# dluvizon/deephar

Hardware: NVIDIA H100
Metric: frames/sec (256x256, 16-frame clips, b32) (higher is better)
Workload: dtype bf16x3 split (fp32 accumulate, wgmma)

## Files before the change

### deephar_b200/csrc/conv_patch.cu

```cuda
#include "tc_common.cuh"

namespace tcd {
using namespace tc;
using R = tc::Roles<2>;
constexpr int WARP_EPI0 = R::WARP_EPI0, WARP_TMA = R::WARP_TMA, WARP_PATCH = R::WARP_PATCH, NTHREADS = R::NTHREADS,
              REGS_PROD = R::REGS_PROD, REGS_EPI = R::REGS_EPI, REGS_CTRL = R::REGS_CTRL;

constexpr int A_BYTES = BM * 64;
constexpr int NWG = 128;
constexpr int NA = 4;
constexpr int NB = 3;
constexpr int MAX_NP = 8;

struct PatchParams {
    TcParams t;
    int np, patch_stride, patch_bytes;
    int ntaps, ncb;
    int tw;
    int ry, fn;
    int pc, pr;
    int rows_per_frame;
    int kw;
    int pt, pl, sh, sw;
    int vh, vw;
    int mask;
};

template <bool LO>
__global__ void __launch_bounds__(NTHREADS, 1)
patch_dense_kernel(const __grid_constant__ PatchParams PP, const __grid_constant__ CUtensorMap map_hi,
                   const __grid_constant__ CUtensorMap map_lo, const __grid_constant__ CUtensorMap map_x) {
    const TcParams& P = PP.t;
    extern __shared__ __align__(1024) uint8_t smem_raw[];
    if (smem_u32(smem_raw) & 1023u) __trap();
    uint8_t* smem = smem_raw;
    const int tid = threadIdx.x;
    const int warp = tid >> 5, lane = tid & 31;
    constexpr bool want_lo = LO;
    const int b_bytes = P.bn_cta * 64;
    uint8_t* b_ring = smem + NA * 2 * A_BYTES;
    uint8_t* patch0 = b_ring + NB * 2 * b_bytes;
    uint64_t* bars = reinterpret_cast<uint64_t*>(patch0 + (size_t)PP.np * PP.patch_stride);
    constexpr int NB_A = NA + 2 * NA;
    constexpr int NB_P = NB_A + 2 * NB;
    const uint32_t bar_full0 = smem_u32(bars), bar_empty0 = smem_u32(bars + NA), bar_fullb0 = smem_u32(bars + NB_A),
                   bar_emptyb0 = smem_u32(bars + NB_A + NB), bar_pfull0 = smem_u32(bars + NB_P),
                   bar_pempty0 = smem_u32(bars + NB_P + MAX_NP);
    const int n0 = blockIdx.y * P.bn_cta;
    const int nkb = P.n_kblocks;
    const int ntaps = PP.ntaps, ncb = PP.ncb, np = PP.np;

    if (warp == WARP_TMA && lane == 0) {
        tma_prefetch_desc(&map_hi);
        if (want_lo) tma_prefetch_desc(&map_lo);
        tma_prefetch_desc(&map_x);
        for (int s = 0; s < NA; ++s) {
            mbar_init(bar_full0 + 8 * s, (uint32_t)NWG);
            mbar_init(bar_empty0 + 16 * s, (uint32_t)R::EPQ);
            mbar_init(bar_empty0 + 16 * s + 8, (uint32_t)R::EPQ);
        }
        for (int s = 0; s < NB; ++s) {
            mbar_init(bar_fullb0 + 8 * s, 1);
            mbar_init(bar_emptyb0 + 8 * s, R::EPQ);
        }
        for (int s = 0; s < MAX_NP; ++s) {
            mbar_init(bar_pfull0 + 8 * s, 1);
            mbar_init(bar_pempty0 + 8 * s, ntaps == 1 ? (uint32_t)NWG : (uint32_t)(2 * NWG));
        }
        fence_barrier_init();
    }
    __syncthreads();

    const int tiles_mine = ((int)P.n_mtiles - (int)blockIdx.x + (int)gridDim.x - 1) / (int)gridDim.x;
    const int total_g = tiles_mine * nkb;
    const int n_patches = tiles_mine * ncb;
    const int rows_per_tile = BM / PP.tw;

    if (warp < WARP_EPI0) {
        reg_prod<REGS_PROD, R::LAUNCH_REGS>();
        const ConvParams& c = P.c;
        const int w = warp >> 2;
        const int tw = tid & (NWG - 1);
        const int ch4 = tw & 7;
        const int prow = tw >> 3;
        uint32_t poff[8];
        int yy[8], xx[8];
// ... 74 lines not shown
                asm volatile("st.shared.v2.b32 [%0], {%1, %2};" ::"r"(a_hi + aoff[i]), "r"(h0), "r"(h1) : "memory");
                if (want_lo) asm volatile("st.shared.v2.b32 [%0], {%1, %2};" ::"r"(a_lo + aoff[i]), "r"(l0), "r"(l1) : "memory");
            }
            const bool last_of_patch = tap + 2 >= ntaps;
            if (last_of_patch) mbar_arrive(bar_pempty0 + 8 * slot);
            fence_proxy_async();
            mbar_arrive(bar_full0 + 8 * s);
            s += 2;
            if (s >= NA) { s -= NA; ++it; }
            tap += 2;
            kx += 2;
            while (tap >= ntaps) {
                tap -= ntaps;
                ++p;
                if (++cb == ncb) { cb = 0; ++ti; }
                if (++slot == np) { slot = 0; pphase ^= 1u; }
                ky = 0; kx = tap;
                if (kx >= PP.kw) { kx -= PP.kw; ky = 1; }
            }
            while (kx >= PP.kw) { kx -= PP.kw; ++ky; }
        }
    } else if (warp < WARP_TMA) {
        reg_inc<REGS_EPI>();
        const int wg = (warp - WARP_EPI0) >> 2, wt = tid - 32 * WARP_EPI0 - 128 * wg;
        float acc[R::MH][ACC_N];
        const uint64_t dbase = make_desc64(smem_u32(smem) + (uint32_t)(wg * 64 * 64));
        const uint64_t dbase_b = make_desc64(smem_u32(b_ring));
        const uint32_t sta16 = (2 * A_BYTES) >> 4, stb16 = (uint32_t)(2 * b_bytes) >> 4, alo16 = A_BYTES >> 4,
                       blo16 = (uint32_t)b_bytes >> 4;
        for (int ti = 0; ti < tiles_mine; ++ti) {
            const int g0 = ti * nkb;
            wg_tile<R::MH, SBK / 16, LO>(
                P.bn_cta, acc, nkb, 0u, alo16, blo16, true,
                [&](int kb, uint64_t& da, uint64_t& db) {
                    const int g = g0 + kb, s = g % NA, sb = g % NB;
                    mbar_wait(bar_full0 + 8 * s, (uint32_t)(g / NA) & 1);
                    mbar_wait(bar_fullb0 + 8 * sb, (uint32_t)(g / NB) & 1);
                    da = dbase + (uint64_t)((uint32_t)s * sta16);
                    db = dbase_b + (uint64_t)((uint32_t)sb * stb16);
                },
                [&](int kb) {
                    const int g = g0 + kb, s = g % NA;
                    wg_release<false>(bar_empty0 + 16 * s + 8 * ((g / NA) & 1), wg, wt, 0u);
                    if (wt == 0) mbar_arrive(bar_emptyb0 + 8 * (g % NB));
                });
            wg_epilogue<R::MH>(P, acc, ((int)blockIdx.x + ti * (int)gridDim.x) * BM + 64 * wg, n0, wt);
        }
    } else {
        reg_dec<REGS_CTRL>();
        if (warp == WARP_TMA) {
            if (lane == 0) {
                const uint32_t tx = (uint32_t)(want_lo ? 2 : 1) * (uint32_t)b_bytes;
                for (int g = 0; g < total_g; ++g) {
                    const int p = g / ntaps, tap = g - p * ntaps;
                    const int cb = p % ncb;
                    const int kc = tap * P.c.Cin + cb * SBK;
                    const int sb = g % NB;
                    const uint32_t itb = (uint32_t)(g / NB);
                    if (itb >= 1) mbar_wait_relaxed(bar_emptyb0 + 8 * sb, (itb - 1) & 1, 0u);
                    const uint32_t full = bar_fullb0 + 8 * sb;
                    mbar_arrive_expect_tx(full, tx);
                    const uint32_t b_hi = smem_u32(b_ring + (size_t)sb * (2 * b_bytes));
                    const uint32_t b_lo = b_hi + (uint32_t)b_bytes;
                    tma_load_2d(b_hi, &map_hi, kc, n0, full);
                    if (want_lo) tma_load_2d(b_lo, &map_lo, kc, n0, full);
                }
            }
        } else if (warp == WARP_PATCH) {
            if (lane == 0) {
// ... 39 lines not shown
    if (!(p.W == 128 || p.W == 64 || p.W == 32 || p.W == 16 || p.W == 8)) return false;
    const int tr = tc::BM / p.W;
    if (tr <= p.H ? (p.H % tr) != 0 : (tr % p.H) != 0) return false;
    g->tw = p.W;
    g->ry = tr <= p.H ? tr : p.H;
    g->fn = tr <= p.H ? 1 : tr / p.H;
    g->pc = p.W + p.kw - 1;
    g->pr = g->ry + p.kh - 1;
    g->rows_per_frame = p.H; g->vh = p.H; g->vw = p.W; g->vn = p.N;
    g->pt = p.pt; g->pl = p.pl; g->kw = p.kw; g->ntaps = p.kh * p.kw;
    g->w_stride = (int64_t)p.ldx * 4; g->h_stride = (int64_t)p.W * p.ldx * 4; g->n_stride = (int64_t)p.H * g->h_stride;
    return true;
}

template <bool LO>
static cudaError_t launch_patch(const PatchParams& PP, const CUtensorMap& map_hi, const CUtensorMap& map_lo,
                                const CUtensorMap& map_x, dim3 grid, size_t smem, cudaStream_t s) {
    cudaError_t e = tc::ensure_smem<patch_dense_kernel<LO>>(smem);
    if (e == cudaSuccess) patch_dense_kernel<LO><<<grid, NTHREADS, smem, s>>>(PP, map_hi, map_lo, map_x);
    return e;
}

static size_t fixed_smem(int bn_cta) {
    return (size_t)NA * 2 * A_BYTES + (size_t)NB * 2 * bn_cta * 64 + 512;
}

}

bool dh_patch_supported(const dh_ctx* ctx, const ConvParams& p, const dh_packed_w* packed) {
    using namespace tcd;
    if (!ctx->dense_patch) return false;
    if (!packed || !packed->hi || !packed->lo) return false;
    if (p.M < 1) return false;
    if ((p.Cin & 7) || (p.ldx & 3) || (reinterpret_cast<uintptr_t>(p.x) & 15)) return false;
    if (p.pre_scale && ((reinterpret_cast<uintptr_t>(p.pre_scale) & 15) || (reinterpret_cast<uintptr_t>(p.pre_shift) & 15)))
        return false;
    const int K = p.kh * p.kw * p.Cin;
    if (packed->k != dh_tc_k_pad(K) || packed->cout_pad != dh_tc_cout_pad(p.Cout)) return false;
    Geom g;
    if (!plan_geom(p, &g)) return false;
    if (g.pc > 256 || g.pr > 256 || g.fn > 256) return false;
    int bn_cta, gy;
    tc::tile_n(p.Cout, &bn_cta, &gy);
    const size_t patch = (size_t)tc::SBK * 4 * g.pc * g.pr * g.fn;
    const size_t stride = (patch + 1023) / 1024 * 1024;
    if (fixed_smem(bn_cta) + 2 * stride > 227 * 1024) return false;
    if ((g.w_stride & 15) || g.n_stride >= (1ll << 40)) return false;
// ... 70 lines not shown
```

### deephar_b200/csrc/conv_sep.cu

```cuda
#include "tc_common.cuh"

namespace tcs {
using namespace tc;
using R = tc::Roles<2, 1>;
constexpr int WARP_EPI0 = R::WARP_EPI0, WARP_TMA = R::WARP_TMA, WARP_PATCH = R::WARP_PATCH, NTHREADS = R::NTHREADS,
              REGS_PROD = R::REGS_PROD, REGS_EPI = R::REGS_EPI, REGS_CTRL = R::REGS_CTRL;

constexpr int A_BYTES = BM * 64;
constexpr int NWG = 128;
constexpr int NPW = 1;
constexpr int NA = 4;
constexpr int NB = 3;
constexpr int NP = 3;

struct SepParams {
    TcParams t;
    int patch_stride;
    int patch_bytes;
    int ry, fn;
    int dbg;
};

template <int KS, int TW, bool SHARE, bool BNPRO, bool LO>
__global__ void __launch_bounds__(NTHREADS, 1)
sep_tma_kernel(const __grid_constant__ SepParams SP, const __grid_constant__ CUtensorMap map_hi,
               const __grid_constant__ CUtensorMap map_lo, const __grid_constant__ CUtensorMap map_x) {
    constexpr int PAD = KS / 2;
    constexpr int PC = TW + 2 * PAD;
    constexpr int NR = 4 + KS - 1;
#ifdef DH_ABLATE
    const int DBG = SP.dbg;
#else
    constexpr int DBG = 0;
#endif
    const TcParams& P = SP.t;
    extern __shared__ __align__(1024) uint8_t smem_raw[];
    if (smem_u32(smem_raw) & 1023u) __trap();
    uint8_t* smem = smem_raw;
    const int tid = threadIdx.x;
    const int warp = tid >> 5, lane = tid & 31;
    constexpr bool want_lo = LO;
    const int b_bytes = P.bn_cta * 64;
    uint8_t* b_ring = smem + NA * 2 * A_BYTES;
    uint8_t* patch0 = b_ring + NB * 2 * b_bytes;
    uint64_t* bars = reinterpret_cast<uint64_t*>(patch0 + NP * SP.patch_stride);
    constexpr int NB_A = NA + 2 * NA;
    const uint32_t bar_full0 = smem_u32(bars), bar_empty0 = smem_u32(bars + NA), bar_fullb0 = smem_u32(bars + NB_A),
                   bar_emptyb0 = smem_u32(bars + NB_A + NB), bar_pfull0 = smem_u32(bars + NB_A + 2 * NB),
                   bar_pempty0 = smem_u32(bars + NB_A + 2 * NB + NP);
    const int n0 = blockIdx.y * P.bn_cta;
    const int nkb = P.n_kblocks;
    const uint32_t my_rank = SHARE ? cluster_ctarank() : 0u;

    if (warp == WARP_TMA && lane == 0) {
        tma_prefetch_desc(&map_hi);
        if (want_lo) tma_prefetch_desc(&map_lo);
        tma_prefetch_desc(&map_x);
        for (int s = 0; s < NA; ++s) {
            mbar_init(bar_full0 + 8 * s, SHARE ? 1u : (uint32_t)NWG);
            mbar_init(bar_empty0 + 16 * s, (SHARE ? 2u : 1u) * R::EPQ);
            mbar_init(bar_empty0 + 16 * s + 8, (SHARE ? 2u : 1u) * R::EPQ);
        }
        for (int s = 0; s < NB; ++s) {
            mbar_init(bar_fullb0 + 8 * s, 1);
            mbar_init(bar_emptyb0 + 8 * s, R::EPQ);
        }
        for (int s = 0; s < NP; ++s) {
            mbar_init(bar_pfull0 + 8 * s, 1);
            mbar_init(bar_pempty0 + 8 * s, NWG);
        }
        fence_barrier_init();
    }
    if (SHARE) cluster_sync_all(); else __syncthreads();

    const int tiles_mine = ((int)P.n_mtiles - (int)blockIdx.x + (int)gridDim.x - 1) / (int)gridDim.x;
    const int total_g = tiles_mine * nkb;
    const int n_own = SHARE ? (total_g - (int)my_rank + 1) / 2 : total_g;

    if (warp < WARP_EPI0) {
        reg_prod<REGS_PROD, R::LAUNCH_REGS>();
        const ConvParams& c = P.c;
        const int w = warp >> 2;
        const int tw = tid & (NWG - 1);
        const int cp = tw & 15;
        const int blk = tw >> 4;
        constexpr int XB = TW / 4;
        const int strip = blk / XB, xb = blk - strip * XB;
        const int fn = (strip * 4) / SP.ry, ry = (strip * 4) - fn * SP.ry;
// ... 94 lines not shown
                    split2(acc[o][q].x, acc[o][q].y, hi, lo);
                    const uint32_t off = swz64(row0 + o * TW + q, cp * 2);
                    *reinterpret_cast<uint32_t*>(a_hi + off) = hi;
                    if (want_lo) *reinterpret_cast<uint32_t*>(a_lo + off) = lo;
                }
            fence_proxy_async();
            if (SHARE) {
                asm volatile("bar.sync %0, %1;" ::"r"(1 + w), "r"(NWG) : "memory");
                if (tw == 0) {
                    mbar_arrive(bar_full0 + 8 * s);
                    const uint32_t peer = my_rank ^ 1u;
                    const uint32_t peer_full = mapa_peer(bar_full0 + 8 * s, peer);
                    if (!(DBG & 8)) {
                        bulk_s2peer(mapa_peer(smem_u32(a_hi), peer), smem_u32(a_hi), A_BYTES, peer_full);
                        if (want_lo) bulk_s2peer(mapa_peer(smem_u32(a_lo), peer), smem_u32(a_lo), A_BYTES, peer_full);
                    }
                }
            } else {
                mbar_arrive(bar_full0 + 8 * s);
            }
        }
    } else if (warp < WARP_TMA) {
        reg_inc<REGS_EPI>();
        const int wg = (warp - WARP_EPI0) >> 2, wt = tid - 32 * WARP_EPI0 - 128 * wg;
        float acc[R::MH][ACC_N];
        const uint64_t dbase = make_desc64(smem_u32(smem) + (uint32_t)(wg * 64 * 64));
        const uint64_t dbase_b = make_desc64(smem_u32(b_ring));
        const uint32_t sta16 = (2 * A_BYTES) >> 4, stb16 = (uint32_t)(2 * b_bytes) >> 4, alo16 = A_BYTES >> 4,
                       blo16 = (uint32_t)b_bytes >> 4;
        for (int ti = 0; ti < tiles_mine; ++ti) {
            const int g0 = ti * nkb;
            wg_tile<R::MH, SBK / 16, LO>(
                P.bn_cta, acc, nkb, 0u, alo16, blo16, !(DBG & 64),
                [&](int kb, uint64_t& da, uint64_t& db) {
                    const int g = g0 + kb, s = g % NA, sb = g % NB;
                    if (!(DBG & 128)) mbar_wait(bar_full0 + 8 * s, (uint32_t)(g / NA) & 1);
                    mbar_wait(bar_fullb0 + 8 * sb, (uint32_t)(g / NB) & 1);
                    da = dbase + (uint64_t)((uint32_t)s * sta16);
                    db = dbase_b + (uint64_t)((uint32_t)sb * stb16);
                },
                [&](int kb) {
                    const int g = g0 + kb, s = g % NA;
                    wg_release<SHARE>(bar_empty0 + 16 * s + 8 * ((g / NA) & 1), wg, wt, my_rank ^ 1u);
                    if (wt == 0) mbar_arrive(bar_emptyb0 + 8 * (g % NB));
                });
            wg_epilogue<R::MH>(P, acc, ((int)blockIdx.x + ti * (int)gridDim.x) * BM + 64 * wg, n0, wt);
        }
    } else {
        reg_dec<REGS_CTRL>();
        if (warp == WARP_TMA) {
            if (lane == 0) {
                const uint32_t tx = (DBG & 16) ? 0u : (uint32_t)(want_lo ? 2 : 1) * (uint32_t)b_bytes;
                const uint32_t tx_a = (DBG & 8) ? 0u : (uint32_t)(want_lo ? 2 : 1) * (uint32_t)A_BYTES;
                for (int g = 0; g < total_g; ++g) {
                    const int ti = g / nkb, kb = g - ti * nkb;
                    const int sb = g % NB;
                    const uint32_t itb = (uint32_t)(g / NB);
                    if (itb >= 1) mbar_wait_relaxed(bar_emptyb0 + 8 * sb, (itb - 1) & 1, (DBG & 2048) ? 64u : 0u);
                    const uint32_t full = bar_fullb0 + 8 * sb;
                    mbar_arrive_expect_tx(full, tx);
                    const uint32_t b_hi = smem_u32(b_ring + (size_t)sb * (2 * b_bytes));
                    const uint32_t b_lo = b_hi + (uint32_t)b_bytes;
                    if (!(DBG & 16)) {
                        tma_load_2d(b_hi, &map_hi, kb * SBK, n0, full);
                        if (want_lo) tma_load_2d(b_lo, &map_lo, kb * SBK, n0, full);
                    }
                    if (SHARE && (uint32_t)(g & 1) != my_rank) {
                        const int sa = g % NA;
                        wait_stage_free(bar_empty0, sa, (uint32_t)(g / NA));
// ... 72 lines not shown
    P.c.K = p.Cin;
    P.k_pad = packed->k;
    P.n_kblocks = p.Cin / SBK;
    int gy;
    tile_n(p.Cout, &P.bn_cta, &gy);
    P.precision = (precision == 1) ? 1 : 3;
    P.ks = p.kh;
    P.n_mtiles = (p.M + BM - 1) / BM;
    P.stages = 2;
    const int pad = p.kh / 2;
    const int tr = BM / p.W;
    SP.ry = tr <= p.H ? tr : p.H;
    SP.fn = tr <= p.H ? 1 : tr / p.H;
    const int pc = p.W + 2 * pad, prr = SP.ry + 2 * pad;
    SP.patch_bytes = SBK * 4 * pc * prr * SP.fn;
    SP.patch_stride = (SP.patch_bytes + 1023) / 1024 * 1024;
#ifdef DH_ABLATE
    SP.dbg = ctx->dbg;
    P.dbg = ctx->dbg;
#else
    SP.dbg = 0;
    P.dbg = 0;
#endif
    const size_t smem = (size_t)NA * 2 * A_BYTES + (size_t)NB * 2 * P.bn_cta * 64 + NP * (size_t)SP.patch_stride + 512;
    if (smem > 227 * 1024) {
        dh_set_error("dh_launch_sep_tma: tile does not fit shared memory");
        return -1;
    }
    CUtensorMap map_hi, map_lo, map_x;
    if (!make_map_b64(&map_hi, packed->hi, packed->k, packed->cout_pad, P.bn_cta) ||
        !make_map_b64(&map_lo, packed->lo, packed->k, packed->cout_pad, P.bn_cta) ||
        !make_map_x(&map_x, p, pc, prr, SP.fn)) {
        dh_set_error("dh_launch_sep_tma: cuTensorMapEncodeTiled failed");
        return -1;
    }
    int gx = ctx->num_sms / gy;
    if (gx < 1) gx = 1;
    if (gx > P.n_mtiles) gx = P.n_mtiles;
    dim3 grid(gx, gy);
    const bool share = gy % 2 == 0 && ctx->share_a;
    cudaError_t e = cudaSuccess;
#define DH_SEP_LAUNCH_(KS_, TW_, BN_, LO_)                                                                              \
    do {                                                                                                         \
        if (share) {                                                                                             \
            e = ensure_smem<sep_tma_kernel<KS_, TW_, true, BN_, LO_>>(smem); \
            if (e == cudaSuccess) {                                                                              \
                cudaLaunchConfig_t cfg = {};                                                                     \
// ... 29 lines not shown
```

### deephar_b200/csrc/conv_tc.cu

```cuda
#include "tc_common.cuh"

namespace tc {
using R = tc::Roles<1>;
constexpr int WARP_EPI0 = R::WARP_EPI0, WARP_TMA = R::WARP_TMA, NTHREADS = R::NTHREADS,
              REGS_PROD = R::REGS_PROD, REGS_EPI = R::REGS_EPI, REGS_CTRL = R::REGS_CTRL;

struct DenseRows {
    int base[8];
    int yx[8];
};

__device__ __forceinline__ void dense_rows_init(const ConvParams& c, int m0, int tid, DenseRows& R) {
    const int HoWo = c.Ho * c.Wo;
#pragma unroll
    for (int i = 0; i < 8; ++i) {
        const int m = m0 + (tid >> 4) + i * 16;
        if (m < c.M) {
            int n = m / HoWo;
            int rem = m - n * HoWo;
            int oy = rem / c.Wo;
            int ox = rem - oy * c.Wo;
            R.base[i] = n * c.H * c.W;
            R.yx[i] = ((oy * c.sh - c.pt) << 16) | ((ox * c.sw - c.pl) & 0xffff);
        } else {
// ... 209 lines not shown
            *reinterpret_cast<uint32_t*>(a_hi + off) = hi;
            if (want_lo) *reinterpret_cast<uint32_t*>(a_lo + off) = lo;
        }
}

__device__ __forceinline__ void dense_load_any(const TcParams& P, const DenseRows& R, int kb, int tid, DenseRegs& D) {
    if (P.ks < 0) dense_load_scalar(P, R, kb, tid, D);
    else dense_load(P, R, kb, tid, D);
}

template <int MODE, bool SHARE, bool LO>
__global__ void __launch_bounds__(NTHREADS, 1)
conv_tc_kernel(const __grid_constant__ TcParams P, const __grid_constant__ CUtensorMap map_hi,
               const __grid_constant__ CUtensorMap map_lo) {
    extern __shared__ __align__(1024) uint8_t smem_raw[];
    if (smem_u32(smem_raw) & 1023u) __trap();
    uint8_t* smem = smem_raw;
    const int tid = threadIdx.x;
    const int warp = tid >> 5, lane = tid & 31;
    constexpr bool want_lo = LO;
    const int b_tile_bytes = P.bn_cta * 128;
    const int stage_bytes = 2 * A_TILE_BYTES + 2 * b_tile_bytes;
    uint64_t* bars = reinterpret_cast<uint64_t*>(smem + (size_t)P.stages * stage_bytes);
    const uint32_t bar_full0 = smem_u32(bars), bar_empty0 = smem_u32(bars + MAX_STAGES);
    const int n0 = blockIdx.y * P.bn_cta;
    const int nkb = P.n_kblocks;

    if (warp == WARP_TMA && lane == 0) {
        tma_prefetch_desc(&map_hi);
        if (want_lo) tma_prefetch_desc(&map_lo);
        for (int s = 0; s < P.stages; ++s) {
            if (SHARE) {
                mbar_init(bar_full0 + 8 * s, (uint32_t)(s & 1) == cluster_ctarank() ? 2u : 1u);
                mbar_init(bar_empty0 + 8 * s, 2 * R::EPQ);
            } else {
                mbar_init(bar_full0 + 8 * s, NPROD + 1);
                mbar_init(bar_empty0 + 8 * s, R::EPQ);
            }
        }
        fence_barrier_init();
    }
    if (SHARE) cluster_sync_all(); else __syncthreads();
    const uint32_t my_rank = SHARE ? cluster_ctarank() : 0u;

    if (warp < WARP_EPI0) {
        reg_prod<REGS_PROD, R::LAUNCH_REGS>();
// ... 45 lines not shown
                uint8_t* a_lo = a_hi + A_TILE_BYTES;
                if (MODE == 0) {
                    dense_store(P, cur, a_hi, a_lo, tid, want_lo);
                    cur = nxt;
                } else if (MODE == 3) produce_sep<3>(P, kb, a_hi, a_lo, m0, tid, want_lo);
                else produce_sep<5>(P, kb, a_hi, a_lo, m0, tid, want_lo);
                fence_proxy_async();
                if (SHARE) {
                    asm volatile("bar.sync 1, %0;" ::"r"(NPROD) : "memory");
                    if (tid == 0) {
                        mbar_arrive(bar_full0 + 8 * s);
                        const uint32_t peer = my_rank ^ 1u;
                        const uint32_t peer_full = mapa_peer(bar_full0 + 8 * s, peer);
                        bulk_s2peer(mapa_peer(smem_u32(a_hi), peer), smem_u32(a_hi), A_TILE_BYTES, peer_full);
                        if (want_lo) bulk_s2peer(mapa_peer(smem_u32(a_lo), peer), smem_u32(a_lo), A_TILE_BYTES, peer_full);
                    }
                } else {
                    mbar_arrive(bar_full0 + 8 * s);
                }
            }
        }
    } else if (warp < WARP_TMA) {
        reg_inc<REGS_EPI>();
        const int wt = tid - 32 * WARP_EPI0;
        float acc[R::MH][ACC_N];
        const uint64_t dbase = make_desc(smem_u32(smem));
        const uint32_t st16 = (uint32_t)stage_bytes >> 4, alo16 = A_TILE_BYTES >> 4, b16 = (2 * A_TILE_BYTES) >> 4,
                       blo16 = (uint32_t)b_tile_bytes >> 4, half16 = (64 * 128) >> 4;
        int s = 0, sr = 0;
        uint32_t it = 0;
        for (int t = blockIdx.x; t < P.n_mtiles; t += gridDim.x) {
            wg_tile<R::MH, BK / 16, LO>(
                P.bn_cta, acc, nkb, half16, alo16, blo16, true,
                [&](int, uint64_t& da, uint64_t& db) {
                    mbar_wait(bar_full0 + 8 * s, it & 1);
                    da = dbase + (uint64_t)((uint32_t)s * st16);
                    db = da + b16;
                    if (++s == P.stages) { s = 0; ++it; }
                },
                [&](int) {
                    wg_release<SHARE>(bar_empty0 + 8 * sr, 0, wt, my_rank ^ 1u);
                    if (++sr == P.stages) sr = 0;
                });
            wg_epilogue<R::MH>(P, acc, t * BM, n0, wt);
        }
    } else {
        reg_dec<REGS_CTRL>();
        if (warp == WARP_TMA) {
            if (lane == 0) {
                const uint32_t tx = (uint32_t)(want_lo ? 2 : 1) * (uint32_t)b_tile_bytes;
                const uint32_t tx_a = (uint32_t)(want_lo ? 2 : 1) * (uint32_t)A_TILE_BYTES;
                int g = 0;
                for (int t = blockIdx.x; t < P.n_mtiles; t += gridDim.x) {
                    for (int kb = 0; kb < nkb; ++kb, ++g) {
                        const int s = g % P.stages;
                        const uint32_t it = (uint32_t)(g / P.stages);
                        mbar_wait(bar_empty0 + 8 * s, (it & 1) ^ 1);
                        const uint32_t full = bar_full0 + 8 * s;
                        mbar_arrive_expect_tx(full, tx + ((SHARE && (uint32_t)(s & 1) != my_rank) ? tx_a : 0u));
                        const uint32_t b_hi = smem_u32(smem + (size_t)s * stage_bytes + 2 * A_TILE_BYTES);
                        const uint32_t b_lo = b_hi + (uint32_t)b_tile_bytes;
                        tma_load_2d(b_hi, &map_hi, kb * BK, n0, full);
                        if (want_lo) tma_load_2d(b_lo, &map_lo, kb * BK, n0, full);
                    }
                }
            }
        }
// ... 35 lines not shown
}

static bool dh_tc_scalar_gather(const ConvParams& p) {
    return (p.Cin & 3) || (p.ldx & 3) || (reinterpret_cast<uintptr_t>(p.x) & 15) ||
           (p.pre_scale && ((reinterpret_cast<uintptr_t>(p.pre_scale) & 15) || (reinterpret_cast<uintptr_t>(p.pre_shift) & 15)));
}

int dh_launch_conv_tc(dh_ctx* ctx, const ConvParams& p, const dh_packed_w* packed, bool separable, int precision,
                      cudaStream_t s) {
    using namespace tc;
    TcParams P;
    P.c = p;
    const int K = separable ? p.Cin : p.kh * p.kw * p.Cin;
    P.c.K = K;
    P.k_pad = packed->k;
    P.n_kblocks = packed->k / BK;
    int gy;
    tile_n(p.Cout, &P.bn_cta, &gy);
    P.precision = (precision == 1) ? 1 : 3;
    P.ks = separable ? p.kh : (dh_tc_scalar_gather(p) ? -1 : 0);
    P.dbg = 0;
    P.n_mtiles = (p.M + BM - 1) / BM;
    const int stage_bytes = 2 * A_TILE_BYTES + 2 * P.bn_cta * 128;
    const int budget = 227 * 1024 - 256 ;
    int stages = budget / stage_bytes;
    if (stages > MAX_STAGES) stages = MAX_STAGES;
    if (stages > P.n_kblocks) stages = P.n_kblocks;
    const bool share = separable && gy % 2 == 0 && P.n_kblocks >= 2 && stages >= 2 && ctx->share_a;
    if (share) stages = stages >= 4 ? 4 : 2;
    if (stages < 1) {
        dh_set_error("dh_launch_conv_tc: tile does not fit shared memory");
        return -1;
    }
    P.stages = stages;
    const size_t smem = (size_t)stages * stage_bytes + 256;

    CUtensorMap map_hi, map_lo;
    if (!make_map(&map_hi, packed->hi, packed->k, packed->cout_pad, P.bn_cta) ||
        !make_map(&map_lo, packed->lo ? packed->lo : packed->hi, packed->k, packed->cout_pad, P.bn_cta)) {
        dh_set_error("dh_launch_conv_tc: cuTensorMapEncodeTiled failed");
        return -1;
    }
    int gx = ctx->num_sms / gy;
    if (gx < 1) gx = 1;
    if (gx > P.n_mtiles) gx = P.n_mtiles;
    dim3 grid(gx, gy);
    cudaError_t e;
#define DH_TC_LAUNCH_(MODE, LO)                                                                              \
    do {                                                                                                     \
        if (share) {                                                                                         \
            e = ensure_smem<conv_tc_kernel<MODE, true, LO>>(smem); \
            if (e == cudaSuccess) {                                                                          \
                cudaLaunchConfig_t cfg = {};                                                                 \
                cfg.gridDim = grid; cfg.blockDim = dim3(NTHREADS); cfg.dynamicSmemBytes = smem; cfg.stream = s; \
                cudaLaunchAttribute at[1];                                                                   \
                at[0].id = cudaLaunchAttributeClusterDimension;                                              \
                at[0].val.clusterDim.x = 1; at[0].val.clusterDim.y = 2; at[0].val.clusterDim.z = 1;          \
                cfg.attrs = at; cfg.numAttrs = 1;                                                            \
// ... 20 lines not shown
```

### deephar_b200/csrc/tc_common.cuh

```cuda
#pragma once
#include <cuda.h>
#include <cuda_bf16.h>
#include "common.cuh"
#include "conv_params.cuh"

namespace tc {


constexpr int BM = 128;
constexpr int BK = 64;
constexpr int NPROD = 256;
constexpr int MAX_BN_CTA = 96;
constexpr int ACC_N = MAX_BN_CTA / 2;
template <int Q, int NPW = 2>
struct Roles {
    static constexpr int EPQ = Q;
    static constexpr int MH = 2 / Q;
    static constexpr int NEPI = 128 * Q;
    static constexpr int WARP_EPI0 = 4 * NPW;
    static constexpr int WARP_TMA = WARP_EPI0 + 4 * Q, WARP_PATCH = WARP_TMA + 2;
    static constexpr int NTHREADS = 32 * (WARP_TMA + 4);
    static constexpr int REGS_PROD = Q == 1 ? 168 : (NPW == 1 ? 192 : 80), REGS_EPI = 144, REGS_CTRL = 32;
    static constexpr int LAUNCH_REGS = NTHREADS <= 512 ? 128 : 96;
    static_assert(128 * NPW * REGS_PROD + NEPI * REGS_EPI + 128 * REGS_CTRL <= NTHREADS * LAUNCH_REGS,
                  "setmaxnreg budget exceeds the CTA's register allocation: the last setmaxnreg.inc would never return");
};
constexpr int A_TILE_BYTES = BM * 128;
constexpr int MAX_STAGES = 4;

struct TcParams {
    ConvParams c;
    int n_kblocks;
    int bn_cta;
    int stages;
    int precision;
    int ks;
    int k_pad;
    int n_mtiles;
    int dbg;
};

__device__ __forceinline__ uint32_t smem_u32(const void* p) { return (uint32_t)__cvta_generic_to_shared(p); }

__device__ __forceinline__ void mbar_init(uint32_t bar, uint32_t count) {
    asm volatile("mbarrier.init.shared::cta.b64 [%0], %1;" ::"r"(bar), "r"(count));
// ... 145 lines not shown
__device__ __forceinline__ void tma_prefetch_4d(const CUtensorMap* map, int c0, int c1, int c2, int c3) {
    asm volatile("cp.async.bulk.prefetch.tensor.4d.L2.global [%0, {%1, %2, %3, %4}];"
                 ::"l"(map), "r"(c0), "r"(c1), "r"(c2), "r"(c3) : "memory");
}

__device__ __forceinline__ uint64_t make_desc64(uint32_t smem_addr) {
    return (uint64_t)((smem_addr >> 4) & 0x3FFF) | (1ull << 16) | ((uint64_t)(512 >> 4) << 32) | (2ull << 62);
}
__device__ __forceinline__ uint32_t swz64(int row, int k) {
    return (uint32_t)(row * 64 + ((((k >> 3) ^ ((row >> 1) & 3)) << 4) | ((k & 7) << 1)));
}

__device__ __forceinline__ float4 lds128(uint32_t a) {
    float4 v;
    asm volatile("ld.shared.v4.f32 {%0, %1, %2, %3}, [%4];" : "=f"(v.x), "=f"(v.y), "=f"(v.z), "=f"(v.w) : "r"(a) : "memory");
    return v;
}

__device__ __forceinline__ void wait_stage_free(uint32_t bar_empty0, int s, uint32_t it, uint32_t ns = 0) {
    if (it >= 1) mbar_wait_relaxed(bar_empty0 + 16 * s + 8 * ((it - 1) & 1), ((it - 1) >> 1) & 1, ns);
}


template <int N, int MH>
__device__ __forceinline__ void acc_fence_all(float (&acc)[MH][ACC_N]) {
#pragma unroll
    for (int h = 0; h < MH; ++h)
#pragma unroll
        for (int i = 0; i < N / 2; ++i) acc_fence(acc[h][i]);
}

template <int N, int MH, int NK16, bool LO>
__device__ __forceinline__ void wg_issue_kblock(float (&acc)[MH][ACC_N], uint64_t da, uint32_t a_half16, uint32_t alo16,
                                                uint64_t db, uint32_t blo16, bool first) {
    wgmma_fence();
#pragma unroll
    for (int k = 0; k < NK16; ++k) {
        const uint32_t acc0 = (first && k == 0) ? 0u : 1u;
#pragma unroll
        for (int h = 0; h < MH; ++h) {
            const uint64_t a = da + (uint64_t)(h * a_half16 + 2 * k);
            wgmma_bf16<N>(acc[h], a, db + 2 * k, acc0);
            if (LO) {
                wgmma_bf16<N>(acc[h], a + alo16, db + 2 * k, 1u);
                wgmma_bf16<N>(acc[h], a, db + blo16 + 2 * k, 1u);
            }
        }
    }
    wgmma_commit();
}

template <int N, int MH, int NK16, bool LO, class Stage, class Release>
__device__ __forceinline__ void wg_tile_n(float (&acc)[MH][ACC_N], int nkb, uint32_t a_half16, uint32_t alo16,
                                          uint32_t blo16, bool mma, Stage& stage, Release& release) {
    for (int kb = 0; kb < nkb; ++kb) {
        uint64_t da, db;
        stage(kb, da, db);
        if (mma) {
            acc_fence_all<N>(acc);
            wg_issue_kblock<N, MH, NK16, LO>(acc, da, a_half16, alo16, db, blo16, kb == 0);
        }
        wgmma_wait<1>();
        acc_fence_all<N>(acc);
        if (kb > 0) release(kb - 1);
    }
    wgmma_wait<0>();
    acc_fence_all<N>(acc);
    release(nkb - 1);
}

template <int MH, int NK16, bool LO, class Stage, class Release>
__device__ __forceinline__ void wg_tile(int bn, float (&acc)[MH][ACC_N], int nkb, uint32_t a_half16, uint32_t alo16,
                                        uint32_t blo16, bool mma, Stage&& stage, Release&& release) {
    switch (bn) {
    case 16: wg_tile_n<16, MH, NK16, LO>(acc, nkb, a_half16, alo16, blo16, mma, stage, release); break;
    case 32: wg_tile_n<32, MH, NK16, LO>(acc, nkb, a_half16, alo16, blo16, mma, stage, release); break;
    case 48: wg_tile_n<48, MH, NK16, LO>(acc, nkb, a_half16, alo16, blo16, mma, stage, release); break;
    case 64: wg_tile_n<64, MH, NK16, LO>(acc, nkb, a_half16, alo16, blo16, mma, stage, release); break;
    case 80: wg_tile_n<80, MH, NK16, LO>(acc, nkb, a_half16, alo16, blo16, mma, stage, release); break;
    default: wg_tile_n<96, MH, NK16, LO>(acc, nkb, a_half16, alo16, blo16, mma, stage, release); break;
    }
}

template <bool SHARE>
__device__ __forceinline__ void wg_release(uint32_t bar, int wg, int wt, uint32_t peer) {
    asm volatile("bar.sync %0, 128;" ::"r"(4 + wg) : "memory");
    if (wt == 0) {
        mbar_arrive(bar);
        if (SHARE) mbar_arrive_cluster(mapa_peer(bar, peer));
    }
}

__device__ __forceinline__ size_t res1_src(const ConvParams& c, int m) {
    if (!c.up1) return (size_t)m;
    const int hw = c.Ho * c.Wo;
    const int n = m / hw, rem = m - n * hw;
    const int y = rem / c.Wo, x = rem - y * c.Wo;
    return ((size_t)n * (c.Ho >> 1) + (y >> 1)) * (size_t)(c.Wo >> 1) + (size_t)(x >> 1);
}

__device__ __forceinline__ float2 ldg2(const float* p) { return __ldg(reinterpret_cast<const float2*>(p)); }

template <int MH>
__device__ __forceinline__ void wg_epilogue(const TcParams& P, const float (&acc)[MH][ACC_N], int m0, int n0, int wt) {
    const ConvParams& c = P.c;
#ifdef DH_ABLATE
    if (P.dbg & 32) return;
#endif
    const int rq = 16 * (wt >> 5) + ((wt & 31) >> 2);
    const int cq = 2 * (wt & 3);
    const bool v2 = !((c.ldo | c.Cout) & 1) && !(reinterpret_cast<uintptr_t>(c.out) & 7) &&
                    (!c.res0 || (!(c.ldr0 & 1) && !(reinterpret_cast<uintptr_t>(c.res0) & 7))) &&
                    (!c.res1 || (!(c.ldr1 & 1) && !(reinterpret_cast<uintptr_t>(c.res1) & 7))) &&
                    (!c.post_scale || (!(reinterpret_cast<uintptr_t>(c.post_scale) & 7) &&
                                       !(reinterpret_cast<uintptr_t>(c.post_shift) & 7)));
    const bool relu = c.post_relu != 0, has_post = c.post_scale != nullptr;
    constexpr int JC = 6;
    static_assert((ACC_N / 4) % JC == 0, "column groups per batch");
#pragma unroll
    for (int h = 0; h < MH; ++h)
#pragma unroll
        for (int hr = 0; hr < 2; ++hr) {
            const int m = m0 + 64 * h + rq + 8 * hr;
            if (m >= c.M) continue;
            float* orow = c.out + (size_t)m * c.ldo;
            const float* r0row = c.res0 ? c.res0 + (size_t)m * c.ldr0 : nullptr;
            const float* r1row = c.res1 ? c.res1 + res1_src(c, m) * c.ldr1 : nullptr;
            if (MH == 1 && v2) {
#pragma unroll
                for (int j0 = 0; j0 < ACC_N / 4; j0 += JC) {
                    if (8 * j0 >= P.bn_cta) break;
                    float2 sc[JC], sh[JC], ra[JC], rb[JC];
#pragma unroll
                    for (int jj = 0; jj < JC; ++jj) {
                        const int co = n0 + 8 * (j0 + jj) + cq;
                        if (8 * (j0 + jj) < P.bn_cta && co < c.Cout) {
                            if (has_post) { sc[jj] = ldg2(c.post_scale + co); sh[jj] = ldg2(c.post_shift + co); }
                            if (r0row) ra[jj] = ldg2(r0row + co);
                            if (r1row) rb[jj] = ldg2(r1row + co);
                        }
                    }
#pragma unroll
                    for (int jj = 0; jj < JC; ++jj) {
                        const int j = j0 + jj;
                        const int co = n0 + 8 * j + cq;
                        if (8 * j < P.bn_cta && co < c.Cout) {
                            float2 v = make_float2(acc[h][4 * j + 2 * hr], acc[h][4 * j + 2 * hr + 1]);
                            if (has_post) v = ffma2(v, sc[jj], sh[jj]);
                            if (relu) v = make_float2(fmaxf(v.x, 0.f), fmaxf(v.y, 0.f));
                            if (r0row) v = fadd2(v, ra[jj]);
                            if (r1row) v = fadd2(v, rb[jj]);
                            *reinterpret_cast<float2*>(orow + co) = v;
                        }
                    }
                }
                continue;
            }
#pragma unroll
            for (int j = 0; j < ACC_N / 4; ++j) {
                if (8 * j >= P.bn_cta) break;
                const int co = n0 + 8 * j + cq;
                float2 v = make_float2(acc[h][4 * j + 2 * hr], acc[h][4 * j + 2 * hr + 1]);
                if (v2) {
                    if (co < c.Cout) {
                        if (has_post) v = ffma2(v, ldg2(c.post_scale + co), ldg2(c.post_shift + co));
                        if (relu) v = make_float2(fmaxf(v.x, 0.f), fmaxf(v.y, 0.f));
                        if (r0row) v = fadd2(v, ldg2(r0row + co));
                        if (r1row) v = fadd2(v, ldg2(r1row + co));
                        *reinterpret_cast<float2*>(orow + co) = v;
                    }
                } else {
#pragma unroll
                    for (int e = 0; e < 2; ++e) {
                        const int cc = co + e;
                        if (cc < c.Cout) {
                            float t = e ? v.y : v.x;
                            if (has_post) t = fmaf(t, __ldg(c.post_scale + cc), __ldg(c.post_shift + cc));
                            if (relu) t = fmaxf(t, 0.f);
                            if (r0row) t += __ldg(r0row + cc);
                            if (r1row) t += __ldg(r1row + cc);
                            orow[cc] = t;
                        }
                    }
                }
            }
        }
}

typedef CUresult (*EncodeTiledFn)(CUtensorMap*, CUtensorMapDataType, cuuint32_t, void*, const cuuint64_t*,
                                  const cuuint64_t*, const cuuint32_t*, const cuuint32_t*, CUtensorMapInterleave,
                                  CUtensorMapSwizzle, CUtensorMapL2promotion, CUtensorMapFloatOOBfill);

static inline EncodeTiledFn get_encode() {
    static EncodeTiledFn fn = nullptr;
    if (!fn) {
        void* p = nullptr;
        cudaDriverEntryPointQueryResult qres;
        if (cudaGetDriverEntryPoint("cuTensorMapEncodeTiled", &p, cudaEnableDefault, &qres) == cudaSuccess &&
            qres == cudaDriverEntryPointSuccess)
            fn = (EncodeTiledFn)p;
    }
    return fn;
}

static inline bool make_map(CUtensorMap* map, const void* base, int k_pad, int rows, int box_rows) {
// ... 44 lines not shown
```

Baseline: 2682.

## Ping-pong consumer warpgroups over whole tiles, stage post-scale in smem, prefetch residuals

The two consumer warpgroups no longer split each 128-row tile in halves. Each now owns alternating whole tiles with MH=2 accumulators and hands off through named barriers, so one warpgroup's epilogue overlaps the other's MMA main loop. Per-channel post scale/shift are staged once into shared memory, residual rows are prefetched into L2 before the tile's MMAs, and the epilogue addressing is simplified. Register budgets are retuned to fit the larger accumulators, which risks spills, and smem grows slightly, which can reduce pipeline stages.

```diff
diff --git a/deephar_b200/csrc/conv_patch.cu b/deephar_b200/csrc/conv_patch.cu
--- a/deephar_b200/csrc/conv_patch.cu
+++ b/deephar_b200/csrc/conv_patch.cu
@@ -41,6 +41,7 @@
     uint8_t* b_ring = smem + NA * 2 * A_BYTES;
     uint8_t* patch0 = b_ring + NB * 2 * b_bytes;
     uint64_t* bars = reinterpret_cast<uint64_t*>(patch0 + (size_t)PP.np * PP.patch_stride);
+    float* post = reinterpret_cast<float*>(bars + 64);
     constexpr int NB_A = NA + 2 * NA;
     constexpr int NB_P = NB_A + 2 * NB;
     const uint32_t bar_full0 = smem_u32(bars), bar_empty0 = smem_u32(bars + NA), bar_fullb0 = smem_u32(bars + NB_A),
@@ -56,12 +57,12 @@
         tma_prefetch_desc(&map_x);
         for (int s = 0; s < NA; ++s) {
             mbar_init(bar_full0 + 8 * s, (uint32_t)NWG);
-            mbar_init(bar_empty0 + 16 * s, (uint32_t)R::EPQ);
-            mbar_init(bar_empty0 + 16 * s + 8, (uint32_t)R::EPQ);
+            mbar_init(bar_empty0 + 16 * s, 1u);
+            mbar_init(bar_empty0 + 16 * s + 8, 1u);
         }
         for (int s = 0; s < NB; ++s) {
             mbar_init(bar_fullb0 + 8 * s, 1);
-            mbar_init(bar_emptyb0 + 8 * s, R::EPQ);
+            mbar_init(bar_emptyb0 + 8 * s, 1);
         }
         for (int s = 0; s < MAX_NP; ++s) {
             mbar_init(bar_pfull0 + 8 * s, 1);
@@ -182,20 +183,24 @@
         }
     } else if (warp < WARP_TMA) {
         reg_inc<REGS_EPI>();
+        stage_post<R::NEPI>(P, n0, post, tid - 32 * WARP_EPI0);
         const int wg = (warp - WARP_EPI0) >> 2, wt = tid - 32 * WARP_EPI0 - 128 * wg;
-        float acc[R::MH][ACC_N];
-        const uint64_t dbase = make_desc64(smem_u32(smem) + (uint32_t)(wg * 64 * 64));
+        float acc[MH][ACC_N];
+        const uint64_t dbase = make_desc64(smem_u32(smem));
         const uint64_t dbase_b = make_desc64(smem_u32(b_ring));
         const uint32_t sta16 = (2 * A_BYTES) >> 4, stb16 = (uint32_t)(2 * b_bytes) >> 4, alo16 = A_BYTES >> 4,
-                       blo16 = (uint32_t)b_bytes >> 4;
-        for (int ti = 0; ti < tiles_mine; ++ti) {
-            const int g0 = ti * nkb;
-            wg_tile<R::MH, SBK / 16, LO>(
-                P.bn_cta, acc, nkb, 0u, alo16, blo16, true,
+                       blo16 = (uint32_t)b_bytes >> 4, half16 = (64 * 64) >> 4;
+        for (int ti = wg; ti < tiles_mine; ti += R::EPQ) {
+            const int g0 = ti * nkb, m0 = ((int)blockIdx.x + ti * (int)gridDim.x) * BM;
+            if (ti > 0) pp_wait(wg);
+            wg_prefetch_res(P, m0, n0, wt);
+            wg_tile<SBK / 16, LO>(
+                P.bn_cta, acc, nkb, half16, alo16, blo16, true,
                 [&](int kb, uint64_t& da, uint64_t& db) {
                     const int g = g0 + kb, s = g % NA, sb = g % NB;
                     mbar_wait(bar_full0 + 8 * s, (uint32_t)(g / NA) & 1);
                     mbar_wait(bar_fullb0 + 8 * sb, (uint32_t)(g / NB) & 1);
+                    if (kb == nkb - 1 && ti + 1 < tiles_mine) pp_pass(wg);
                     da = dbase + (uint64_t)((uint32_t)s * sta16);
                     db = dbase_b + (uint64_t)((uint32_t)sb * stb16);
                 },
@@ -204,7 +209,7 @@
                     wg_release<false>(bar_empty0 + 16 * s + 8 * ((g / NA) & 1), wg, wt, 0u);
                     if (wt == 0) mbar_arrive(bar_emptyb0 + 8 * (g % NB));
                 });
-            wg_epilogue<R::MH>(P, acc, ((int)blockIdx.x + ti * (int)gridDim.x) * BM + 64 * wg, n0, wt);
+            wg_epilogue(P, acc, m0, n0, wt, post);
         }
     } else {
         reg_dec<REGS_CTRL>();
@@ -290,7 +295,7 @@
 }
 
 static size_t fixed_smem(int bn_cta) {
-    return (size_t)NA * 2 * A_BYTES + (size_t)NB * 2 * bn_cta * 64 + 512;
+    return (size_t)NA * 2 * A_BYTES + (size_t)NB * 2 * bn_cta * 64 + 512 + POST_SMEM;
 }
 
 }
diff --git a/deephar_b200/csrc/conv_sep.cu b/deephar_b200/csrc/conv_sep.cu
--- a/deephar_b200/csrc/conv_sep.cu
+++ b/deephar_b200/csrc/conv_sep.cu
@@ -44,6 +44,7 @@
     uint8_t* b_ring = smem + NA * 2 * A_BYTES;
     uint8_t* patch0 = b_ring + NB * 2 * b_bytes;
     uint64_t* bars = reinterpret_cast<uint64_t*>(patch0 + NP * SP.patch_stride);
+    float* post = reinterpret_cast<float*>(bars + 64);
     constexpr int NB_A = NA + 2 * NA;
     const uint32_t bar_full0 = smem_u32(bars), bar_empty0 = smem_u32(bars + NA), bar_fullb0 = smem_u32(bars + NB_A),
                    bar_emptyb0 = smem_u32(bars + NB_A + NB), bar_pfull0 = smem_u32(bars + NB_A + 2 * NB),
@@ -58,12 +59,12 @@
         tma_prefetch_desc(&map_x);
         for (int s = 0; s < NA; ++s) {
             mbar_init(bar_full0 + 8 * s, SHARE ? 1u : (uint32_t)NWG);
-            mbar_init(bar_empty0 + 16 * s, (SHARE ? 2u : 1u) * R::EPQ);
-            mbar_init(bar_empty0 + 16 * s + 8, (SHARE ? 2u : 1u) * R::EPQ);
+            mbar_init(bar_empty0 + 16 * s, SHARE ? 2u : 1u);
+            mbar_init(bar_empty0 + 16 * s + 8, SHARE ? 2u : 1u);
         }
         for (int s = 0; s < NB; ++s) {
             mbar_init(bar_fullb0 + 8 * s, 1);
-            mbar_init(bar_emptyb0 + 8 * s, R::EPQ);
+            mbar_init(bar_emptyb0 + 8 * s, 1);
         }
         for (int s = 0; s < NP; ++s) {
             mbar_init(bar_pfull0 + 8 * s, 1);
@@ -204,20 +205,24 @@
         }
     } else if (warp < WARP_TMA) {
         reg_inc<REGS_EPI>();
+        stage_post<R::NEPI>(P, n0, post, tid - 32 * WARP_EPI0);
         const int wg = (warp - WARP_EPI0) >> 2, wt = tid - 32 * WARP_EPI0 - 128 * wg;
-        float acc[R::MH][ACC_N];
-        const uint64_t dbase = make_desc64(smem_u32(smem) + (uint32_t)(wg * 64 * 64));
+        float acc[MH][ACC_N];
+        const uint64_t dbase = make_desc64(smem_u32(smem));
         const uint64_t dbase_b = make_desc64(smem_u32(b_ring));
         const uint32_t sta16 = (2 * A_BYTES) >> 4, stb16 = (uint32_t)(2 * b_bytes) >> 4, alo16 = A_BYTES >> 4,
-                       blo16 = (uint32_t)b_bytes >> 4;
-        for (int ti = 0; ti < tiles_mine; ++ti) {
-            const int g0 = ti * nkb;
-            wg_tile<R::MH, SBK / 16, LO>(
-                P.bn_cta, acc, nkb, 0u, alo16, blo16, !(DBG & 64),
+                       blo16 = (uint32_t)b_bytes >> 4, half16 = (64 * 64) >> 4;
+        for (int ti = wg; ti < tiles_mine; ti += R::EPQ) {
+            const int g0 = ti * nkb, m0 = ((int)blockIdx.x + ti * (int)gridDim.x) * BM;
+            if (ti > 0) pp_wait(wg);
+            wg_prefetch_res(P, m0, n0, wt);
+            wg_tile<SBK / 16, LO>(
+                P.bn_cta, acc, nkb, half16, alo16, blo16, !(DBG & 64),
                 [&](int kb, uint64_t& da, uint64_t& db) {
                     const int g = g0 + kb, s = g % NA, sb = g % NB;
                     if (!(DBG & 128)) mbar_wait(bar_full0 + 8 * s, (uint32_t)(g / NA) & 1);
                     mbar_wait(bar_fullb0 + 8 * sb, (uint32_t)(g / NB) & 1);
+                    if (kb == nkb - 1 && ti + 1 < tiles_mine) pp_pass(wg);
                     da = dbase + (uint64_t)((uint32_t)s * sta16);
                     db = dbase_b + (uint64_t)((uint32_t)sb * stb16);
                 },
@@ -226,7 +231,7 @@
                     wg_release<SHARE>(bar_empty0 + 16 * s + 8 * ((g / NA) & 1), wg, wt, my_rank ^ 1u);
                     if (wt == 0) mbar_arrive(bar_emptyb0 + 8 * (g % NB));
                 });
-            wg_epilogue<R::MH>(P, acc, ((int)blockIdx.x + ti * (int)gridDim.x) * BM + 64 * wg, n0, wt);
+            wg_epilogue(P, acc, m0, n0, wt, post);
         }
     } else {
         reg_dec<REGS_CTRL>();
@@ -345,7 +350,8 @@
     SP.dbg = 0;
     P.dbg = 0;
 #endif
-    const size_t smem = (size_t)NA * 2 * A_BYTES + (size_t)NB * 2 * P.bn_cta * 64 + NP * (size_t)SP.patch_stride + 512;
+    const size_t smem = (size_t)NA * 2 * A_BYTES + (size_t)NB * 2 * P.bn_cta * 64 + NP * (size_t)SP.patch_stride + 512 +
+                        POST_SMEM;
     if (smem > 227 * 1024) {
         dh_set_error("dh_launch_sep_tma: tile does not fit shared memory");
         return -1;
diff --git a/deephar_b200/csrc/conv_tc.cu b/deephar_b200/csrc/conv_tc.cu
--- a/deephar_b200/csrc/conv_tc.cu
+++ b/deephar_b200/csrc/conv_tc.cu
@@ -255,6 +255,7 @@
     const int b_tile_bytes = P.bn_cta * 128;
     const int stage_bytes = 2 * A_TILE_BYTES + 2 * b_tile_bytes;
     uint64_t* bars = reinterpret_cast<uint64_t*>(smem + (size_t)P.stages * stage_bytes);
+    float* post = reinterpret_cast<float*>(bars + 32);
     const uint32_t bar_full0 = smem_u32(bars), bar_empty0 = smem_u32(bars + MAX_STAGES);
     const int n0 = blockIdx.y * P.bn_cta;
     const int nkb = P.n_kblocks;
@@ -346,15 +347,16 @@
         }
     } else if (warp < WARP_TMA) {
         reg_inc<REGS_EPI>();
+        stage_post<R::NEPI>(P, n0, post, tid - 32 * WARP_EPI0);
         const int wt = tid - 32 * WARP_EPI0;
-        float acc[R::MH][ACC_N];
+        float acc[MH][ACC_N];
         const uint64_t dbase = make_desc(smem_u32(smem));
         const uint32_t st16 = (uint32_t)stage_bytes >> 4, alo16 = A_TILE_BYTES >> 4, b16 = (2 * A_TILE_BYTES) >> 4,
                        blo16 = (uint32_t)b_tile_bytes >> 4, half16 = (64 * 128) >> 4;
         int s = 0, sr = 0;
         uint32_t it = 0;
         for (int t = blockIdx.x; t < P.n_mtiles; t += gridDim.x) {
-            wg_tile<R::MH, BK / 16, LO>(
+            wg_tile<BK / 16, LO>(
                 P.bn_cta, acc, nkb, half16, alo16, blo16, true,
                 [&](int, uint64_t& da, uint64_t& db) {
                     mbar_wait(bar_full0 + 8 * s, it & 1);
@@ -366,7 +368,7 @@
                     wg_release<SHARE>(bar_empty0 + 8 * sr, 0, wt, my_rank ^ 1u);
                     if (++sr == P.stages) sr = 0;
                 });
-            wg_epilogue<R::MH>(P, acc, t * BM, n0, wt);
+            wg_epilogue(P, acc, t * BM, n0, wt, post);
         }
     } else {
         reg_dec<REGS_CTRL>();
@@ -448,7 +450,7 @@
     P.dbg = 0;
     P.n_mtiles = (p.M + BM - 1) / BM;
     const int stage_bytes = 2 * A_TILE_BYTES + 2 * P.bn_cta * 128;
-    const int budget = 227 * 1024 - 256 ;
+    const int budget = 227 * 1024 - 256  - POST_SMEM;
     int stages = budget / stage_bytes;
     if (stages > MAX_STAGES) stages = MAX_STAGES;
     if (stages > P.n_kblocks) stages = P.n_kblocks;
@@ -459,7 +461,7 @@
         return -1;
     }
     P.stages = stages;
-    const size_t smem = (size_t)stages * stage_bytes + 256;
+    const size_t smem = (size_t)stages * stage_bytes + 256 + POST_SMEM;
 
     CUtensorMap map_hi, map_lo;
     if (!make_map(&map_hi, packed->hi, packed->k, packed->cout_pad, P.bn_cta) ||
diff --git a/deephar_b200/csrc/tc_common.cuh b/deephar_b200/csrc/tc_common.cuh
--- a/deephar_b200/csrc/tc_common.cuh
+++ b/deephar_b200/csrc/tc_common.cuh
@@ -12,15 +12,16 @@
 constexpr int NPROD = 256;
 constexpr int MAX_BN_CTA = 96;
 constexpr int ACC_N = MAX_BN_CTA / 2;
+constexpr int MH = BM / 64;
 template <int Q, int NPW = 2>
 struct Roles {
     static constexpr int EPQ = Q;
-    static constexpr int MH = 2 / Q;
     static constexpr int NEPI = 128 * Q;
     static constexpr int WARP_EPI0 = 4 * NPW;
     static constexpr int WARP_TMA = WARP_EPI0 + 4 * Q, WARP_PATCH = WARP_TMA + 2;
     static constexpr int NTHREADS = 32 * (WARP_TMA + 4);
-    static constexpr int REGS_PROD = Q == 1 ? 168 : (NPW == 1 ? 192 : 80), REGS_EPI = 144, REGS_CTRL = 32;
+    static constexpr int REGS_PROD = Q == 1 ? 168 : (NPW == 1 ? 192 : 88);
+    static constexpr int REGS_EPI = Q == 2 && NPW == 2 ? 136 : 144, REGS_CTRL = 32;
     static constexpr int LAUNCH_REGS = NTHREADS <= 512 ? 128 : 96;
     static_assert(128 * NPW * REGS_PROD + NEPI * REGS_EPI + 128 * REGS_CTRL <= NTHREADS * LAUNCH_REGS,
                   "setmaxnreg budget exceeds the CTA's register allocation: the last setmaxnreg.inc would never return");
@@ -212,7 +213,7 @@
 }
 
 
-template <int N, int MH>
+template <int N>
 __device__ __forceinline__ void acc_fence_all(float (&acc)[MH][ACC_N]) {
 #pragma unroll
     for (int h = 0; h < MH; ++h)
@@ -220,7 +221,7 @@
         for (int i = 0; i < N / 2; ++i) acc_fence(acc[h][i]);
 }
 
-template <int N, int MH, int NK16, bool LO>
+template <int N, int NK16, bool LO>
 __device__ __forceinline__ void wg_issue_kblock(float (&acc)[MH][ACC_N], uint64_t da, uint32_t a_half16, uint32_t alo16,
                                                 uint64_t db, uint32_t blo16, bool first) {
     wgmma_fence();
@@ -240,7 +241,7 @@
     wgmma_commit();
 }
 
-template <int N, int MH, int NK16, bool LO, class Stage, class Release>
+template <int N, int NK16, bool LO, class Stage, class Release>
 __device__ __forceinline__ void wg_tile_n(float (&acc)[MH][ACC_N], int nkb, uint32_t a_half16, uint32_t alo16,
                                           uint32_t blo16, bool mma, Stage& stage, Release& release) {
     for (int kb = 0; kb < nkb; ++kb) {
@@ -248,7 +249,7 @@
         stage(kb, da, db);
         if (mma) {
             acc_fence_all<N>(acc);
-            wg_issue_kblock<N, MH, NK16, LO>(acc, da, a_half16, alo16, db, blo16, kb == 0);
+            wg_issue_kblock<N, NK16, LO>(acc, da, a_half16, alo16, db, blo16, kb == 0);
         }
         wgmma_wait<1>();
         acc_fence_all<N>(acc);
@@ -259,18 +260,21 @@
     release(nkb - 1);
 }
 
-template <int MH, int NK16, bool LO, class Stage, class Release>
+template <int NK16, bool LO, class Stage, class Release>
 __device__ __forceinline__ void wg_tile(int bn, float (&acc)[MH][ACC_N], int nkb, uint32_t a_half16, uint32_t alo16,
                                         uint32_t blo16, bool mma, Stage&& stage, Release&& release) {
     switch (bn) {
-    case 16: wg_tile_n<16, MH, NK16, LO>(acc, nkb, a_half16, alo16, blo16, mma, stage, release); break;
-    case 32: wg_tile_n<32, MH, NK16, LO>(acc, nkb, a_half16, alo16, blo16, mma, stage, release); break;
-    case 48: wg_tile_n<48, MH, NK16, LO>(acc, nkb, a_half16, alo16, blo16, mma, stage, release); break;
-    case 64: wg_tile_n<64, MH, NK16, LO>(acc, nkb, a_half16, alo16, blo16, mma, stage, release); break;
-    case 80: wg_tile_n<80, MH, NK16, LO>(acc, nkb, a_half16, alo16, blo16, mma, stage, release); break;
-    default: wg_tile_n<96, MH, NK16, LO>(acc, nkb, a_half16, alo16, blo16, mma, stage, release); break;
-    }
-}
+    case 16: wg_tile_n<16, NK16, LO>(acc, nkb, a_half16, alo16, blo16, mma, stage, release); break;
+    case 32: wg_tile_n<32, NK16, LO>(acc, nkb, a_half16, alo16, blo16, mma, stage, release); break;
+    case 48: wg_tile_n<48, NK16, LO>(acc, nkb, a_half16, alo16, blo16, mma, stage, release); break;
+    case 64: wg_tile_n<64, NK16, LO>(acc, nkb, a_half16, alo16, blo16, mma, stage, release); break;
+    case 80: wg_tile_n<80, NK16, LO>(acc, nkb, a_half16, alo16, blo16, mma, stage, release); break;
+    default: wg_tile_n<96, NK16, LO>(acc, nkb, a_half16, alo16, blo16, mma, stage, release); break;
+    }
+}
+
+__device__ __forceinline__ void pp_pass(int wg) { asm volatile("bar.arrive %0, 256;" ::"r"(6 + wg) : "memory"); }
+__device__ __forceinline__ void pp_wait(int wg) { asm volatile("bar.sync %0, 256;" ::"r"(7 - wg) : "memory"); }
 
 template <bool SHARE>
 __device__ __forceinline__ void wg_release(uint32_t bar, int wg, int wt, uint32_t peer) {
@@ -291,21 +295,57 @@
 
 __device__ __forceinline__ float2 ldg2(const float* p) { return __ldg(reinterpret_cast<const float2*>(p)); }
 
-template <int MH>
-__device__ __forceinline__ void wg_epilogue(const TcParams& P, const float (&acc)[MH][ACC_N], int m0, int n0, int wt) {
+constexpr int POST_SMEM = 2 * MAX_BN_CTA * 4;
+template <int NEPI>
+__device__ __forceinline__ void stage_post(const TcParams& P, int n0, float* post, int ct) {
+    const ConvParams& c = P.c;
+    if (c.post_scale) {
+        for (int j = ct; j < P.bn_cta; j += NEPI) {
+            const int co = n0 + j;
+            post[j] = co < c.Cout ? __ldg(c.post_scale + co) : 0.f;
+            post[MAX_BN_CTA + j] = co < c.Cout ? __ldg(c.post_shift + co) : 0.f;
+        }
+    }
+    asm volatile("bar.sync 2, %0;" ::"n"(NEPI) : "memory");
+}
+
+__device__ __forceinline__ void prefetch_l2(const float* p) { asm volatile("prefetch.global.L2 [%0];" ::"l"(p)); }
+__device__ __forceinline__ void wg_prefetch_res(const TcParams& P, int m0, int n0, int wt) {
+    const ConvParams& c = P.c;
+#ifdef DH_ABLATE
+    if (P.dbg & 32) return;
+#endif
+    const int m = m0 + wt;
+    if (m >= c.M) return;
+    const int last = min(P.bn_cta, c.Cout - n0) - 1;
+    if (c.res0) {
+        const float* r = c.res0 + (size_t)m * c.ldr0 + n0;
+        for (int k = 0; k < last; k += 32) prefetch_l2(r + k);
+        prefetch_l2(r + last);
+    }
+    if (c.res1) {
+        const float* r = c.res1 + res1_src(c, m) * c.ldr1 + n0;
+        for (int k = 0; k < last; k += 32) prefetch_l2(r + k);
+        prefetch_l2(r + last);
+    }
+}
+
+__device__ __forceinline__ void wg_epilogue(const TcParams& P, const float (&acc)[MH][ACC_N], int m0, int n0, int wt,
+                                            const float* post) {
     const ConvParams& c = P.c;
 #ifdef DH_ABLATE
     if (P.dbg & 32) return;
 #endif
     const int rq = 16 * (wt >> 5) + ((wt & 31) >> 2);
-    const int cq = 2 * (wt & 3);
+    const int c0 = n0 + 2 * (wt & 3);
     const bool v2 = !((c.ldo | c.Cout) & 1) && !(reinterpret_cast<uintptr_t>(c.out) & 7) &&
                     (!c.res0 || (!(c.ldr0 & 1) && !(reinterpret_cast<uintptr_t>(c.res0) & 7))) &&
-                    (!c.res1 || (!(c.ldr1 & 1) && !(reinterpret_cast<uintptr_t>(c.res1) & 7))) &&
-                    (!c.post_scale || (!(reinterpret_cast<uintptr_t>(c.post_scale) & 7) &&
-                                       !(reinterpret_cast<uintptr_t>(c.post_shift) & 7)));
+                    (!c.res1 || (!(c.ldr1 & 1) && !(reinterpret_cast<uintptr_t>(c.res1) & 7)));
     const bool relu = c.post_relu != 0, has_post = c.post_scale != nullptr;
-    constexpr int JC = 6;
+    const int ncol = min(P.bn_cta - 2 * (wt & 3), c.Cout - c0);
+    const float* sc = post + (c0 - n0);
+    const float* sh = sc + MAX_BN_CTA;
+    constexpr int JC = 3;
     static_assert((ACC_N / 4) % JC == 0, "column groups per batch");
 #pragma unroll
     for (int h = 0; h < MH; ++h)
@@ -313,34 +353,33 @@
         for (int hr = 0; hr < 2; ++hr) {
             const int m = m0 + 64 * h + rq + 8 * hr;
             if (m >= c.M) continue;
-            float* orow = c.out + (size_t)m * c.ldo;
-            const float* r0row = c.res0 ? c.res0 + (size_t)m * c.ldr0 : nullptr;
-            const float* r1row = c.res1 ? c.res1 + res1_src(c, m) * c.ldr1 : nullptr;
-            if (MH == 1 && v2) {
+            float* orow = c.out + (size_t)m * c.ldo + c0;
+            const float* r0row = c.res0 ? c.res0 + (size_t)m * c.ldr0 + c0 : nullptr;
+            const float* r1row = c.res1 ? c.res1 + res1_src(c, m) * c.ldr1 + c0 : nullptr;
+            if (v2) {
 #pragma unroll
                 for (int j0 = 0; j0 < ACC_N / 4; j0 += JC) {
                     if (8 * j0 >= P.bn_cta) break;
-                    float2 sc[JC], sh[JC], ra[JC], rb[JC];
+                    float2 ra[JC], rb[JC];
 #pragma unroll
                     for (int jj = 0; jj < JC; ++jj) {
-                        const int co = n0 + 8 * (j0 + jj) + cq;
-                        if (8 * (j0 + jj) < P.bn_cta && co < c.Cout) {
-                            if (has_post) { sc[jj] = ldg2(c.post_scale + co); sh[jj] = ldg2(c.post_shift + co); }
-                            if (r0row) ra[jj] = ldg2(r0row + co);
-                            if (r1row) rb[jj] = ldg2(r1row + co);
+                        if (8 * (j0 + jj) < ncol) {
+                            if (r0row) ra[jj] = ldg2(r0row + 8 * (j0 + jj));
+                            if (r1row) rb[jj] = ldg2(r1row + 8 * (j0 + jj));
                         }
                     }
 #pragma unroll
                     for (int jj = 0; jj < JC; ++jj) {
                         const int j = j0 + jj;
-                        const int co = n0 + 8 * j + cq;
-                        if (8 * j < P.bn_cta && co < c.Cout) {
+                        if (8 * j < ncol) {
                             float2 v = make_float2(acc[h][4 * j + 2 * hr], acc[h][4 * j + 2 * hr + 1]);
-                            if (has_post) v = ffma2(v, sc[jj], sh[jj]);
+                            if (has_post)
+                                v = ffma2(v, *reinterpret_cast<const float2*>(sc + 8 * j),
+                                          *reinterpret_cast<const float2*>(sh + 8 * j));
                             if (relu) v = make_float2(fmaxf(v.x, 0.f), fmaxf(v.y, 0.f));
                             if (r0row) v = fadd2(v, ra[jj]);
                             if (r1row) v = fadd2(v, rb[jj]);
-                            *reinterpret_cast<float2*>(orow + co) = v;
+                            *reinterpret_cast<float2*>(orow + 8 * j) = v;
                         }
                     }
                 }
@@ -349,28 +388,16 @@
 #pragma unroll
             for (int j = 0; j < ACC_N / 4; ++j) {
                 if (8 * j >= P.bn_cta) break;
-                const int co = n0 + 8 * j + cq;
-                float2 v = make_float2(acc[h][4 * j + 2 * hr], acc[h][4 * j + 2 * hr + 1]);
-                if (v2) {
-                    if (co < c.Cout) {
-                        if (has_post) v = ffma2(v, ldg2(c.post_scale + co), ldg2(c.post_shift + co));
-                        if (relu) v = make_float2(fmaxf(v.x, 0.f), fmaxf(v.y, 0.f));
-                        if (r0row) v = fadd2(v, ldg2(r0row + co));
-                        if (r1row) v = fadd2(v, ldg2(r1row + co));
-                        *reinterpret_cast<float2*>(orow + co) = v;
-                    }
-                } else {
-#pragma unroll
-                    for (int e = 0; e < 2; ++e) {
-                        const int cc = co + e;
-                        if (cc < c.Cout) {
-                            float t = e ? v.y : v.x;
-                            if (has_post) t = fmaf(t, __ldg(c.post_scale + cc), __ldg(c.post_shift + cc));
-                            if (relu) t = fmaxf(t, 0.f);
-                            if (r0row) t += __ldg(r0row + cc);
-                            if (r1row) t += __ldg(r1row + cc);
-                            orow[cc] = t;
-                        }
+#pragma unroll
+                for (int e = 0; e < 2; ++e) {
+                    const int k = 8 * j + e;
+                    if (k < ncol) {
+                        float t = acc[h][4 * j + 2 * hr + e];
+                        if (has_post) t = fmaf(t, sc[k], sh[k]);
+                        if (relu) t = fmaxf(t, 0.f);
+                        if (r0row) t += __ldg(r0row + k);
+                        if (r1row) t += __ldg(r1row + k);
+                        orow[k] = t;
                     }
                 }
             }
```

New measurement: 2804 (median of 6 runs). 1.05x the previous value.
